# asbschmidt/CUDASW4

Measured on AMD Instinct MI355X. Metric: GCUPS, higher is better.
Workload: dtype f16x2; 1 GPU; peak: allqueries.fasta (20 queries, 41752 residues) vs pseudo DB 1000000 x 512, half2 kernel configuration, blosum62, gop -11 gex -1, top 10, C++ host driver; db_subjects=1000000, db_residues=512000000, queries=20, kernel=half2, queries_in_flight=1, tail_overlaps=10, numa_node_rank0=1, numa_bound=True, resident=True, residency=resident, cached_chars=512000000, parallelism=db-shard x1 (one DB sharded), one top-K gather per step + host merge

## Files before the change

cudasw4_amd/csrc/sw_api.hip:

```cpp
#include <hip/hip_runtime.h>
#include <hipcub/hipcub.hpp>

#include <algorithm>
#include <cstdio>
#include <cmath>
#include <cstdlib>
#include <cstring>
#include <ctime>
#include <string>
#include <vector>

#include "../../include/cudasw4_amd.h"
#include "../../include/cudasw4_amd_engine.h"
#include "../../include/cudasw4_amd_pssm.h"
#include "sw_internal.hpp"
#include "sw_launch.hpp"
#include "sw_pssm.hpp"
#include "sw_rows_pipeline.hpp"

namespace {

thread_local std::string g_last_error = "";

int fail(int code, const std::string& msg) {
// ... 122 lines not shown
    bool have_query = false;
    bool pssm_mode = false;
    int8_t* d_pssm = nullptr;
    size_t pssm_capacity = 0;
    int pssm_max = 1;
    Profile profiles[4][4][3];
    bool use_offs = true;
    int64_t long16_min = -1;
    int64_t long16_min_default = -1;
    int matrix_max = 1;
    bool i32_native = false;
    int32_t lanes4_max_subject = -1;
    int32_t lanes4_max_q = -1;
    int32_t lanes8_max_q = -1;
    bool check_bounds = false;
    uint32_t pipe_spin_limit = 1u << 20;
    int32_t pipe_drop_stage = -1;
    int32_t pipe_cpl = 0;
    int32_t stream_slots = 4;
    int32_t stream_jump = 0;
    int32_t stream_cols_max = 4096;
    int32_t stream_multi_cols_max = 1536;
    int32_t stream_multi_max_subject = -1;
    int32_t pipe_quorum = 0;
    int32_t pipe_slot = 0;
};

namespace {

int score_max(const sw_ctx* ctx) { return std::max(1, ctx->pssm_mode ? ctx->pssm_max : ctx->matrix_max); }
bool have_scores(const sw_ctx* ctx) { return ctx->have_matrix || ctx->pssm_mode; }

int max_grid(const sw_ctx* ctx) {
    const int g = std::max(1, ctx->num_cus) * ctx->grid_mult;
    return ctx->grid_cap > 0 ? std::min(g, ctx->grid_cap) : g;
}

int rescore_lanes(int32_t max_subject_len) { return max_subject_len > 1280 ? 64 : 16; }

int shape_index(int lanes) { return lanes == 64 ? 1 : lanes == 8 ? 2 : lanes == 4 ? 3 : 0; }

int effective_kind_of(const sw_ctx* ctx, int kind, int32_t max_subject_len) {
    if (kind != SW_KIND_I32 || ctx->i32_native || !ctx->have_query) return kind;
    const int64_t bound = (int64_t)std::min(ctx->qlen, max_subject_len) * score_max(ctx) + ((int64_t)1 << 22) + 4096;
    return bound < ((int64_t)1 << 24) ? SW_KIND_F32 : SW_KIND_I32;
}
// ... 39 lines not shown
        pr.dev = nullptr;
        pr.capacity = 0;
        SW_HIP(hipMalloc(&pr.dev, cap));
        pr.capacity = cap;
    }
    if (ctx->pssm_mode) SW_HIP(kl->profile(pl.rows, lanes, nullptr, ctx->qlen, ctx->d_pssm, ctx->qlen, pl.nstripes, pr.dev, shift, frame == 2 ? 1 : 0, stream));
    else SW_HIP(kl->profile(pl.rows, lanes, ctx->d_query, ctx->qlen, ctx->d_matrix, ctx->dim, pl.nstripes, pr.dev, shift, frame == 2 ? 1 : 0, stream));
    pr.shift = shift;
    if (!pr.ready) SW_HIP(hipEventCreateWithFlags(&pr.ready, hipEventDisableTiming));
    SW_HIP(hipEventRecord(pr.ready, stream));
    pr.plan = pl;
    pr.valid = true;
    return SW_OK;
}

int32_t border_capacity(int32_t max_len, int lanes) {
    const int64_t steps = ((int64_t)max_len + lanes - 1 + 3) / 4 * 4;
    return (int32_t)((steps + 15) / 16 * 16 + 16);
}
size_t border_bytes_per_wg(int32_t lcap, int lanes) {
    if (lanes == 4) return 0;
    const size_t region = lanes == 16 ? swk::group_region_words<16>(lcap) : lanes == 8 ? swk::group_region_words<8>(lcap) : swk::group_region_words<64>(lcap);
    return (size_t)(swk::kThreads / lanes) * region * sizeof(uint32_t);
}

__global__ void max_length_kernel(const int32_t* lengths, const int32_t* positions, const int32_t* count_ptr, int32_t first_pos,
                                  int32_t n, int32_t* out) {
    const int32_t cnt = count_ptr ? min(*count_ptr, n) : n;
    int32_t m = 0;
    for (int32_t i = blockIdx.x * blockDim.x + threadIdx.x; i < cnt; i += gridDim.x * blockDim.x)
        m = max(m, lengths[positions ? positions[i] : first_pos + i]);
    if (m > 0) atomicMax(out, m);
}

struct StreamPlan { int slots = 0, cols = 0, room = 0, base = 0, jump = 0; };
StreamPlan stream_plan(const sw_ctx* ctx, int kind, int lanes, int a, const QueryPlan& pl, int32_t max_subject_len) {
    StreamPlan sp;
    if (!kind_packed(kind) || lanes != 16 || a < 0) return sp;
    const bool multi = pl.nstripes > 1;
    const int P = swk::frame_classes(true, pl.rows, lanes, multi);
    sp.base = kind == SW_KIND_F16X2 ? -2016 : 0;
    const int top = kind == SW_KIND_F16X2 ? 1024 : 12400;
    sp.jump = ctx->stream_jump > 0 ? ctx->stream_jump : (kind == SW_KIND_F16X2 ? 512 : 2048);
    sp.room = top - sp.base - a * (2 * lanes + 4 + P);
    sp.cols = a > 0 ? std::min(sp.room / a, ctx->stream_cols_max) : ctx->stream_cols_max;
    sp.slots = std::max(1, std::min(ctx->stream_slots, swk::kStreamMaxSlots));
// ... 135 lines not shown
            p.uniform_frame = 1;
            for (int u = 0; u < swk::kLevelWords; u++)
                p.levels[u] = kind == SW_KIND_F16X2 ? swk::Arith<swk::F16X2>::zero_at(a, std::min<int>(u, (int)K + 16))
                                                    : swk::Arith<swk::I16X2>::zero_at(a, std::min<int>(u, (int)K + 16));
        }
    }
    if (sp.slots >= 1) {
        p.stream_slots = sp.slots; p.stream_cols = sp.cols; p.stream_room = sp.room; p.level_base = sp.base;
        p.jump = sp.jump; p.jump_limit = sp.jump - 4;
        p.jump_word = kind == SW_KIND_F16X2 ? swk::Arith<swk::F16X2>::pos_word(sp.jump) : swk::Arith<swk::I16X2>::pos_word(sp.jump);
    }
    p.scores = scores; p.ids = ids; p.id_offset = id_offset;
    p.ovf_pos = ovf_pos; p.ovf_count = ovf_count; p.ovf_check = (ovf_check && kind_packed(kind)) ? 1 : 0;
    p.scratch = nullptr; p.lcap = 0; p.zeros = ctx->d_zeros + kind * 16;
    p.stat_count = stat_count; p.stat_limit = stat_limit;
    if (multi) {
        p.lcap = border_capacity(max_subject_len, lanes);
        if (p.stream_slots > 1) {
            int cols = p.stream_cols;
            while (cols > max_subject_len && (size_t)grid * border_bytes_per_wg(border_capacity(cols, lanes), lanes) > temp_bytes) cols = cols * 3 / 4;
            p.stream_cols = cols;
            p.lcap = border_capacity(std::max(max_subject_len, cols), lanes);
        }
        const size_t per_wg = border_bytes_per_wg(p.lcap, lanes);
        if (!temp || temp_bytes < per_wg) return fail(SW_ERR_TEMP, "temp buffer too small for a multi-stripe query");
        grid = (int)std::min<size_t>((size_t)grid, temp_bytes / per_wg);
        p.scratch = static_cast<uint32_t*>(temp);
    }
    SW_HIP(take_work_slot(ctx, stream, &p.work_counter));
    p.start_signal = start_signal;
    p.start_quorum = (uint32_t)std::min(grid, 64);
    p.dry_signal = dry_signal;
    if (!stat_count && !positions && p.stream_slots > 1 && lanes == 16 && kind_packed(kind)) { p.stat_count = ctx->dirty_counter; p.stat_limit = INT32_MAX; }
    p.dry_value = ctx->dry_value;
    const int reserve = (list.service_workgroups > 0 || list.claim) ? 0 : ctx->grid_reserve;
    SW_HIP(kl->scan(pl.rows, lanes, multi, offs, grid, reserve, stream, p));
    return SW_OK;
}

}

namespace {
#define SW_REP8(OP) OP(0) OP(1) OP(2) OP(3) OP(4) OP(5) OP(6) OP(7)
#define SW_OP_PK_MAX3(i) asm volatile("v_pk_maximum3_f16 %0, %0, %1, %2" : "+v"(a[i]) : "v"(b), "v"(c));
#define SW_OP_ADD_F32(i) asm volatile("v_add_f32 %0, %0, %1" : "+v"(a[i]) : "v"(b));
#define SW_OP_MAX3_F32(i) asm volatile("v_max3_f32 %0, %0, %1, %2" : "+v"(a[i]) : "v"(b), "v"(c));
#define SW_OP_ADD_U32(i) asm volatile("v_add_u32 %0, %0, %1" : "+v"(a[i]) : "v"(b));
// ... 116 lines not shown
int sw_ctx_create(int device, sw_ctx** out) {
    if (!out) return fail(SW_ERR_INVALID, "null out pointer");
    *out = nullptr;
    int n = 0;
    if (hipGetDeviceCount(&n) != hipSuccess || n <= 0) return fail(SW_ERR_NO_DEVICE, "no HIP device available (this library has no CPU path)");
    if (device < 0 || device >= n) return fail(SW_ERR_INVALID, "device index out of range");
    SW_HIP(hipSetDevice(device));
    hipDeviceProp_t prop;
    SW_HIP(hipGetDeviceProperties(&prop, device));
    sw_ctx* ctx = new sw_ctx;
    ctx->device = device;
    ctx->num_cus = prop.multiProcessorCount;
    if (const char* e = getenv("CUDASW4_AMD_GRID_CAP")) ctx->grid_cap = std::max(0, atoi(e));
    if (const char* e = getenv("CUDASW4_AMD_NO_OFFS")) ctx->use_offs = !(e[0] == '1');
    if (const char* e = getenv("CUDASW4_AMD_I32_NATIVE")) ctx->i32_native = e[0] == '1';
    if (const char* e = getenv("CUDASW4_AMD_LANES8_MAX_Q")) ctx->lanes8_max_q = atoi(e);
    if (const char* e = getenv("CUDASW4_AMD_LANES4_MAX_Q")) ctx->lanes4_max_q = atoi(e);
    if (const char* e = getenv("CUDASW4_AMD_LANES4_MAX_SUBJECT")) ctx->lanes4_max_subject = atoi(e);
    if (const char* e = getenv("CUDASW4_AMD_CHECK_BOUNDS")) ctx->check_bounds = e[0] == '1';
    if (const char* e = getenv("CUDASW4_AMD_PIPE_SPIN_LIMIT")) ctx->pipe_spin_limit = (uint32_t)std::max(1ll, atoll(e));
    if (const char* e = getenv("CUDASW4_AMD_PIPE_TEST_DROP_STAGE")) ctx->pipe_drop_stage = atoi(e);
    if (const char* e = getenv("CUDASW4_AMD_PIPE_CPL")) ctx->pipe_cpl = atoi(e);
    if (const char* e = getenv("CUDASW4_AMD_STREAM")) ctx->stream_slots = std::max(0, std::min(swk::kStreamMaxSlots, atoi(e)));
    hipError_t e = hipMalloc(&ctx->d_matrix, 26 * swk::kLetters);
    if (e == hipSuccess) e = hipMalloc(&ctx->d_zeros, 256 + 64);
    if (e == hipSuccess) e = hipMalloc(&ctx->d_work, 2 * kWorkSlots * sizeof(uint32_t));
    if (e == hipSuccess) {
        uint32_t z[64] = {};
        for (int i = 0; i < 16; i++) z[SW_KIND_I16X2 * 16 + i] = swk::Arith<swk::I16X2>::kZero;
        e = hipMemcpy(ctx->d_zeros, z, sizeof(z), hipMemcpyHostToDevice);
    }
    for (int kind = 0; kind < 4 && e == hipSuccess; kind++) e = kind_launch(kind)->warm(nullptr);
    if (e == hipSuccess) e = hipStreamSynchronize(nullptr);
    if (e != hipSuccess) { delete ctx; return fail(SW_ERR_HIP, std::string("context set-up: ") + hipGetErrorString(e)); }
    *out = ctx;
    return SW_OK;
}

int sw_ctx_destroy(sw_ctx* ctx) {
    if (!ctx) return SW_OK;
    (void)hipSetDevice(ctx->device);
    if (ctx->d_matrix) (void)hipFree(ctx->d_matrix);
    if (ctx->d_zeros) (void)hipFree(ctx->d_zeros);
    if (ctx->d_work) (void)hipFree(ctx->d_work);
    if (ctx->d_query) (void)hipFree(ctx->d_query);
    if (ctx->d_pssm) (void)hipFree(ctx->d_pssm);
// ... 515 lines not shown
    return SW_OK;
}

static size_t scan_temp_bytes_of(sw_ctx* ctx, int kind, int part_id, int32_t n, int32_t max_subject_len);
size_t sw_scan_temp_bytes(sw_ctx* ctx, int kind, int part_id, int32_t n, int32_t max_subject_len) {
    if (!ctx || !ctx->have_query || !kind_launch(kind) || max_subject_len < 0 || n <= 0) return 0;
    if (kind_packed(kind) && part_id >= 0) {
        const int fb = packed_fallback_kind(kind);
        const size_t own = scan_temp_bytes_of(ctx, kind, part_id, n, max_subject_len);
        return std::max(own, scan_temp_bytes_of(ctx, effective_kind_of(ctx, fb, max_subject_len), part_id, n, max_subject_len));
    }
    return scan_temp_bytes_of(ctx, effective_kind_of(ctx, kind, max_subject_len), part_id, n, max_subject_len);
}

static size_t scan_temp_bytes_of(sw_ctx* ctx, int kind, int part_id, int32_t n, int32_t max_subject_len) {
    const int lanes = part_id < 0 ? rescore_lanes(max_subject_len) : lanes_for_partition(ctx, kind, part_id, n, max_subject_len);
    const QueryPlan pl = plan_query(kind, ctx->qlen, lanes);
    if (pl.nstripes <= 1) return 0;
    const int subj_per_batch = (swk::kThreads / lanes) * (kind_packed(kind) ? 2 : 1);
    const int64_t nbatches = ((int64_t)n + subj_per_batch - 1) / subj_per_batch;
    const int64_t grid = std::min<int64_t>(nbatches, max_grid(ctx));
    const StreamPlan sp = stream_plan(ctx, kind, lanes, 1, pl, max_subject_len);
    const int32_t cols = sp.slots > 1 ? std::max(max_subject_len, sp.cols) : max_subject_len;
    return (size_t)grid * border_bytes_per_wg(border_capacity(cols, lanes), lanes);
}

int sw_scan_partition(sw_ctx* ctx, int kind, int part_id, const int8_t* chars, const uint64_t* offsets,
                      const int32_t* lengths, int32_t first_pos, int32_t n, int32_t max_subject_len, int gop, int gex,
                      float* scores, int32_t* ids, int64_t id_offset, int32_t* ovf_pos, int32_t* ovf_count,
                      int ovf_check, void* temp, size_t temp_bytes, void* stream) {
    if (!ctx) return fail(SW_ERR_INVALID, "null context");
    if (part_id < 0 || part_id >= SW_NUM_LENGTH_PARTITIONS || !kind_launch(kind)) {
        ctx->start_signal = nullptr;
        ctx->dry_signal = nullptr;
        return fail(SW_ERR_INVALID, part_id < 0 || part_id >= SW_NUM_LENGTH_PARTITIONS ? "partition id out of range" : "unknown kind");
    }
    kind = effective_kind_of(ctx, kind, max_subject_len);
    int lanes = lanes_for_partition(ctx, kind, part_id, n, max_subject_len);
    if (kind_packed(kind) && !offs_possible(ctx, kind, lanes, max_subject_len, gop, gex, ovf_check, nullptr)) {
        kind = effective_kind_of(ctx, packed_fallback_kind(kind), max_subject_len);
        lanes = lanes_for_partition(ctx, kind, part_id, n, max_subject_len);
        ovf_pos = nullptr; ovf_count = nullptr; ovf_check = 0;
    }
    return scan_common(ctx, kind, lanes, chars, offsets, lengths, nullptr, nullptr, first_pos, n, max_subject_len, gop, gex,
                       scores, ids, id_offset, ovf_pos, ovf_count, ovf_check, temp, temp_bytes,
                       static_cast<hipStream_t>(stream));
// ... 471 lines not shown
```

cudasw4_amd/csrc/sw_dp_kernel.hpp:

```cpp
#pragma once

#include <hip/hip_runtime.h>
#include <stdint.h>

#include <type_traits>

#include "sw_pssm.hpp"

namespace swk {

typedef uint32_t u32;
typedef short s16x2 __attribute__((ext_vector_type(2)));
typedef unsigned short u16x2 __attribute__((ext_vector_type(2)));
typedef _Float16 f16x2 __attribute__((ext_vector_type(2)));

constexpr int kGroup = 16;
constexpr int kThreads = 256;
constexpr int kPadLetter = 20;
constexpr int kLetters = 21;

enum { F16X2 = 0, I16X2 = 1, I32 = 2, F32 = 3 };

constexpr int DPP_ROW_SHL1 = 0x101;
constexpr int DPP_ROW_SHR1 = 0x111;
// ... 261 lines not shown
    int32_t renorm_quads;
    u32 renorm_word;
    u32 wrap_class;
    u32 wrap_last;
    int32_t* stat_count;
    int32_t stat_limit;
    u32* start_signal;
    u32 start_quorum;
    int32_t* claim;
    int32_t service;
    const u32* done_flag;
    u32 done_value;
    u32* dry_signal;
    u32 dry_value;
    int32_t stream_slots;
    int32_t stream_cols;
    int32_t stream_room;
    int32_t level_base;
    int32_t jump;
    u32 jump_word;
    int32_t jump_limit;
    int32_t uniform_frame;
    int32_t flag_period;
    u32 levels[kLevelWords];
};

constexpr int32_t kListEmpty = -1, kListTaken = -2;

typedef u32 u32x3 __attribute__((ext_vector_type(3)));

template <int NW, int CHUNK_ROW_BYTES>
__device__ __forceinline__ void lds_read_chunk(u32 (&dst)[NW], const unsigned char* p, int c) {
    using C = Chunks<NW>;
    const int w = C::first(c);
    if (c < C::kN4) {
        const uint4 v = *reinterpret_cast<const uint4*>(p + c * CHUNK_ROW_BYTES);
        dst[w + 0] = v.x; dst[w + 1] = v.y; dst[w + 2] = v.z; dst[w + 3] = v.w;
    } else if (c < C::kCount) {
        const u32x3 v = *reinterpret_cast<const u32x3*>(p + c * CHUNK_ROW_BYTES);
        if constexpr (C::kSplit) {
            dst[w + 0] = v.x; dst[w + 1] = v.y; dst[w + 2] = v.z;
        } else {
            u32 x = v.x;
            if constexpr (C::kRem == 1) asm("" : "+v"(x) : "v"(v.y), "v"(v.z));
            if constexpr (C::kRem == 2) asm("" : "+v"(x) : "v"(v.z));
            dst[w] = x;
// ... 267 lines not shown
    return v;
}

template <int LANES>
struct Border {
    static constexpr int kBlockCols = 2 * LANES;
    static constexpr int kQuadsPerBlock = LANES / 2;
    static constexpr int kBlockBytes = 8 * kBlockCols;
    static constexpr int kBlockWords = 2 * kBlockCols;
    static constexpr int kInBytes = kBlockBytes, kOutBytes = kBlockBytes, kDummyBytes = 8 * (kThreads / LANES) + 32;
    static constexpr int kGroupBytes = kInBytes + kOutBytes + 16;
    static constexpr int ring_bytes(int groups) { return groups * kGroupBytes + kDummyBytes; }
    static_assert(kGroupBytes % 16 == 0, "rings are read and written 16 bytes at a time");
    static constexpr int blocks(int steps) { return (steps + kBlockCols - 1) / kBlockCols + 3; }
};
template <int LANES>
constexpr int border_region_words(int lcap) { return Border<LANES>::blocks(lcap) * Border<LANES>::kBlockWords; }

template <int LANES>
constexpr int stream_region_words(int lcap) { return LANES == 16 ? Border<LANES>::blocks(lcap) * Border<LANES>::kBlockCols : 0; }
template <int LANES>
constexpr int group_region_words(int lcap) { return border_region_words<LANES>(lcap) + stream_region_words<LANES>(lcap); }

__device__ __forceinline__ void announce_start(const ScanParams& p) {
    if (p.start_signal && threadIdx.x == 0) {
        if (atomicAdd(p.work_counter + 1, 1u) + 1u == p.start_quorum)
            __hip_atomic_fetch_add(p.start_signal, 1u, __ATOMIC_RELEASE, __HIP_MEMORY_SCOPE_SYSTEM);
    }
}

#ifndef SWK_I32_WAVES3_MAX_R
#define SWK_I32_WAVES3_MAX_R 32
#endif
#ifndef SWK_I32_WAVES3_MAX_R_MULTI
#define SWK_I32_WAVES3_MAX_R_MULTI 32
#endif
#ifndef SWK_F32_WAVES3_MAX_R
#define SWK_F32_WAVES3_MAX_R 48
#endif
#ifndef SWK_F32_WAVES3_MAX_R_MULTI
#define SWK_F32_WAVES3_MAX_R_MULTI 48
#endif
constexpr int min_waves_of(int KIND, int R, int LANES, bool MULTI) {
    const bool packed = KIND == F16X2 || KIND == I16X2;
    if (packed && LANES <= 16 && MULTI && R <= SWK_WAVES3_MAX_R_MULTI) return 3;
    if (packed) return (LANES <= 16 && !MULTI && R <= SWK_WAVES4_MAX_R) ? 4 : (LANES <= 16 && !MULTI && R <= SWK_WAVES3_MAX_R) ? 3 : 2;
    if (KIND == I32 && LANES <= 16 && R > (MULTI ? SWK_I32_WAVES3_MAX_R_MULTI : SWK_I32_WAVES3_MAX_R)) return 2;
    if (KIND == F32 && LANES <= 16 && R > (MULTI ? SWK_F32_WAVES3_MAX_R_MULTI : SWK_F32_WAVES3_MAX_R)) return 2;
    return (R <= 16 && !MULTI && LANES <= 16) ? 4 : 3;
}
template <int KIND, int R, int LANES, bool MULTI>
constexpr int min_waves() { return min_waves_of(KIND, R, LANES, MULTI); }
constexpr int vgpr_slot_of(int KIND, int R, int LANES, bool MULTI) { return (512 / min_waves_of(KIND, R, LANES, MULTI)) & ~7; }

template <int KIND, int R, int LANES, bool MULTI, bool OFFS = false>
__global__ void __launch_bounds__(kThreads, (min_waves<KIND, R, LANES, MULTI>())) sw_scan_kernel(const ScanParams p) {
    using A = Arith<KIND>;
    using G = Geometry<KIND, R, LANES>;
    constexpr int kGroups = kThreads / LANES;
    using BD = Border<LANES>;
    constexpr int SHL1 = Shift<LANES>::kShl1;
    constexpr int kQuadsPerLetterBlock = LANES;
    static_assert(!A::kPacked || OFFS, "packed kinds run the column-offset recurrence only (sw_launch.hpp: launch_scan_ro)");
    constexpr bool kUni = A::kPacked;
    constexpr bool kAddr = A::kPacked && MULTI && LANES == 16;
    constexpr int P = OFFS ? frame_classes(A::kPacked, R, LANES, MULTI, kUni) : 1;
    __shared__ __attribute__((aligned(16))) unsigned char lds[16 + G::kTileBytes];
    __shared__ __attribute__((aligned(16))) unsigned char rings[MULTI ? BD::ring_bytes(kGroups) : 16];

    const int tid = threadIdx.x;
    const int lane = tid & (LANES - 1);
    const int group = tid / LANES;
    const bool head = lane == 0;
    const int slot = LANES < 16 ? (tid & 15) : lane;
    const u32 laneStep = kAddr ? 16u * (u32)slot : (A::kPacked ? 0x00100010u : 16u) * ((LANES < 16 && head) ? u32(slot + 1) : 1u);
    announce_start(p);
    if (p.positions) __builtin_amdgcn_s_setprio(2);
    const bool service = p.service != 0;
    const int n = (p.count_ptr && !service) ? *p.count_ptr : p.n;
    constexpr int kSubjPerBatch = kGroups * A::kSubjects;
    const int nbatches = (n + kSubjPerBatch - 1) / kSubjPerBatch;
    if (!service && (int)blockIdx.x >= nbatches) return;

    if constexpr (!MULTI) {
        load_tile<G::kTileBytes>(lds, p.profile);
        __syncthreads();
    }

    unsigned char* const ringIn = rings + (MULTI ? group * BD::kGroupBytes : 0);
    unsigned char* const ringOut = ringIn + BD::kInBytes;
    u32* const gBorder = MULTI ? p.scratch + ((size_t)blockIdx.x * kGroups + group) * (size_t)group_region_words<LANES>(p.lcap) : nullptr;
    typedef const __attribute__((address_space(1))) unsigned char* StreamPtr;
    StreamPtr streamBase = nullptr;
    u32 streamOff = 0;
    if constexpr (kAddr) {
        constexpr int kGroupsPerWave = 64 / LANES;
        const int g0 = group & ~(kGroupsPerWave - 1);
        const uintptr_t b = reinterpret_cast<uintptr_t>(p.scratch + ((size_t)blockIdx.x * kGroups + g0) * (size_t)group_region_words<LANES>(p.lcap) +
                                                        border_region_words<LANES>(p.lcap));
        streamBase = (StreamPtr)(((uintptr_t)(u32)__builtin_amdgcn_readfirstlane((int)(b >> 32)) << 32) |
                                 (uintptr_t)(u32)__builtin_amdgcn_readfirstlane((int)(u32)b));
        streamOff = 4u * (u32)((group - g0) * group_region_words<LANES>(p.lcap) + LANES - lane);
    }

    const u32 apos = OFFS ? A::pos_word(p.gex_mag) : 0u;
// ... 8 lines not shown
        for (int spin = 0; spin < (1 << 20); spin++) {
            const int v = __hip_atomic_load(p.claim + i, __ATOMIC_RELAXED, __HIP_MEMORY_SCOPE_AGENT);
            if (v == kListTaken) return -1;
            if (v >= 0) return atomicCAS(p.claim + i, v, kListTaken) == v ? v : -1;
            __builtin_amdgcn_s_sleep(2);
        }
        return -1;
    };
    for (;;) {
        __syncthreads();
        if (tid == 0) {
            int b = (int)atomicAdd(p.work_counter, 1u), avail = n;
            if (service) {
                avail = 0;
                for (u32 spin = 0; b < nbatches; spin++) {
                    avail = __hip_atomic_load(p.count_ptr, __ATOMIC_RELAXED, __HIP_MEMORY_SCOPE_AGENT);
                    if (avail > b * kSubjPerBatch) break;
                    const u32 done = __hip_atomic_load(p.done_flag, __ATOMIC_RELAXED, __HIP_MEMORY_SCOPE_SYSTEM);
                    if ((int32_t)(done - p.done_value) >= 0 || spin > 600000u) { b = nbatches; break; }
                    __builtin_amdgcn_s_sleep(127);
                }
                avail = min(avail, n);
            }
            if (b == nbatches && p.dry_signal) __hip_atomic_store(p.dry_signal, p.dry_value, __ATOMIC_RELAXED, __HIP_MEMORY_SCOPE_SYSTEM);
            next_batch = b;
            batch_avail = avail;
        }
        __syncthreads();
        const int b = next_batch;
        if (b >= nbatches) break;
        const int navail = batch_avail;
        const int batch = service ? b : nbatches - 1 - b;
        const int i0 = batch * kSubjPerBatch + group * A::kSubjects;
        const int i1 = i0 + 1;
        bool valid0 = i0 < navail;
        bool valid1 = A::kPacked && (i1 < navail);
        int pos0 = 0, pos1 = 0, len0 = 0, len1 = 0;
        const int8_t* s0 = p.chars;
        const int8_t* s1 = p.chars;
        if (p.claim) {
            int v = -1;
            if (valid0 && lane == 0) v = claim_entry(i0);
            if constexpr (LANES == 64) v = __builtin_amdgcn_readfirstlane(v);
            else v = __shfl(v, (tid & 63) & ~(LANES - 1));
            valid0 = v >= 0;
            pos0 = valid0 ? v : 0;
            if (valid0) {
                len0 = p.lengths[pos0];
                s0 = p.chars + (p.offsets[pos0] - p.offsets[0]);
            }
            valid1 = false;
        } else {
            if (valid0) {
                pos0 = p.positions ? p.positions[i0] : p.first_pos + i0;
                len0 = p.lengths[pos0];
                s0 = p.chars + (p.offsets[pos0] - p.offsets[0]);
            }
            if (valid1) {
                pos1 = p.positions ? p.positions[i1] : p.first_pos + i1;
                len1 = p.lengths[pos1];
                s1 = p.chars + (p.offsets[pos1] - p.offsets[0]);
            }
        }
        int lmax = len0 > len1 ? len0 : len1;
        if constexpr (LANES <= 16) {
            if constexpr (LANES <= 4) lmax = max(lmax, __shfl_xor(lmax, 4));
            if constexpr (LANES <= 8) lmax = max(lmax, __shfl_xor(lmax, 8));
            lmax = max(lmax, __shfl_xor(lmax, 16));
            lmax = max(lmax, __shfl_xor(lmax, 32));
        }
        int nquads = (lmax + LANES - 1 + 3) >> 2;
        if constexpr (MULTI) nquads = min(nquads, (p.lcap - 4) >> 2);
        nquads = __builtin_amdgcn_readfirstlane(nquads);
        const int len0pad = (len0 + 3) & ~3, len1pad = (len1 + 3) & ~3;
        auto letters4 = [&](const int8_t* s, int lenpad, int j) -> u32 {
            u32 w = 0x14141414u;
            if (j < lenpad) w = *reinterpret_cast<const u32*>(s + j);
            return w * (u32)G::kLetterUnits;
        };
        if constexpr (kAddr) {
            u32* const sw = gBorder + border_region_words<LANES>(p.lcap) + LANES;
            sw[lane - LANES] = (u32)(kPadLetter * G::kLetterUnits) * 0x01000100u;
            for (int c = lane; c < nquads + LANES / 4; c += LANES) {
                const u32 a = letters4(s0, len0pad, 4 * c), b = letters4(s1, len1pad, 4 * c);
                *reinterpret_cast<uint4*>(sw + 4 * c) = make_uint4(__builtin_amdgcn_perm(b, a, 0x040c000cu), __builtin_amdgcn_perm(b, a, 0x050c010cu),
                                                                   __builtin_amdgcn_perm(b, a, 0x060c020cu), __builtin_amdgcn_perm(b, a, 0x070c030cu));
            }
            __builtin_amdgcn_fence(__ATOMIC_RELEASE, "workgroup");
        }

        u32 maxv = 0u;
        for (int stripe = 0; stripe < p.nstripes; stripe++) {
            const bool first = stripe == 0;
            if constexpr (MULTI) {
                __syncthreads();
                load_tile<G::kTileBytes>(lds, p.profile + (size_t)stripe * G::kTileBytes);
                __syncthreads();
            }
            StripeState<KIND, R, P> st;
            u32 zw[P + 5];
            const int tg0 = kUni ? __builtin_amdgcn_readfirstlane(LANES * stripe) : 0;
            auto load_levels = [&](int q) {
                const int u0 = __builtin_amdgcn_readfirstlane((tg0 + 4 * q) & kmask);
#pragma unroll
                for (int k = 0; k < P + 5; k++) zw[k] = p.levels[u0 + k];
#pragma unroll
                for (int k = 0; k < P + 5; k++) asm volatile("" : "+s"(zw[k]));
            };
            if constexpr (kUni) {
                load_levels(0);
#pragma unroll
                for (int r = 0; r < R; r++) { st.H[r] = zw[r % P]; st.E[r] = zw[r % P + 1]; }
                st.upH_prev = A::gap(zw[(R - 1) % P], p.gex); st.Hlast = zw[(R - 1) % P]; st.Fout = zw[0];
#pragma unroll
                for (int d = 0; d < P + 3; d++) st.maxv[d] = A::add(maxv, zw[d + 1]);
            } else {
                u32 zc[P + 5];
                zc[0] = zbefore; zc[1] = zstart;
#pragma unroll
                for (int k = 2; k < P + 5; k++) zc[k] = A::add(zc[k - 1], apos);
#pragma unroll
                for (int r = 0; r < R; r++) { st.H[r] = zc[r % P]; st.E[r] = zc[r % P + 1]; }
                st.upH_prev = zc[(R - 1) % P]; st.Hlast = zc[(R - 1) % P]; st.Fout = zbefore;
#pragma unroll
                for (int k = 0; k < P + 4; k++) st.Zc[k] = zc[k + 1];
#pragma unroll
                for (int d = 0; d < P + 3; d++) st.maxv[d] = OFFS ? A::add(maxv, zc[A::kWindow ? d + 1 : d]) : maxv;
            }
            st.yA = ((u32)(kPadLetter * G::kLetterUnits) << G::kLetterShift) + 16u * (u32)(slot + 1);
            st.yB = st.yA;
            if constexpr (A::kPacked && LANES <= 16) st.yA |= st.yA << 16;

            auto fetch = [&](const int8_t* s, int lenpad, int blk) -> u32 {
                if constexpr (kAddr) return 0u;
                else return letters4(s, lenpad, blk * (4 * LANES) + lane * 4);
            };
            u32 nextA = fetch(s0, len0pad, 0);
            u32 nextB = A::kPacked ? fetch(s1, len1pad, 0) : 0u;
// ... 105 lines not shown
                        if (lower) lower_frame();
                    }
                    if constexpr (MULTI) *reinterpret_cast<uint2*>(outPtr + 8 * BYTE) = make_uint2(st.Hlast, st.Fout);
                };
                border_step(std::integral_constant<int, 0>{});
                border_step(std::integral_constant<int, 1>{});
                border_step(std::integral_constant<int, 2>{});
                border_step(std::integral_constant<int, 3>{});
                if constexpr (MULTI) outPtr += walkOut;
                if constexpr (!kAddr) {
                    lettersA = dpp<SHL1, true>(0u, lettersA);
                    if constexpr (A::kPacked) lettersB = dpp<SHL1, true>(0u, lettersB);
                }
                if constexpr (OFFS && A::kWindow) {
                    if constexpr (!kUni) {
#pragma unroll
                        for (int k = 0; k < P + 4; k++) st.Zc[k] = A::add(st.Zc[k], apos4);
                    }
#pragma unroll
                    for (int d = 0; d < P + 3; d++) st.maxv[d] = A::add(st.maxv[d], apos4);
                }
                if constexpr (kUni) load_levels(q + 1);
            };
            if constexpr (!MULTI) {
                for (int q = 0; q < nquads; q++) quad(q);
            } else {
                for (int q0 = 0; q0 < nquads; q0 += BD::kQuadsPerBlock) {
                    const int qend = min(nquads, q0 + BD::kQuadsPerBlock);
                    for (int q = q0; q < qend; q++) quad(q);
                    if (qend == q0 + BD::kQuadsPerBlock) block_end(q0 / BD::kQuadsPerBlock);
                }
            }
            if constexpr (MULTI) {
                if (!last) {
                    const int done = nquads & ~(BD::kQuadsPerBlock - 1);
                    const int slot = 4 * (nquads - done) + lane;
                    u32* const g = gBorder + (size_t)(done / BD::kQuadsPerBlock) * BD::kBlockWords;
                    __builtin_amdgcn_fence(__ATOMIC_ACQ_REL, "wavefront");
                    if (slot < BD::kBlockCols) *reinterpret_cast<uint2*>(ringOut + 8 * slot) = make_uint2(A::kZero, A::kZero);
                    else *reinterpret_cast<uint2*>(g + 2 * slot) = make_uint2(A::kZero, A::kZero);
                    __builtin_amdgcn_fence(__ATOMIC_ACQ_REL, "wavefront");
                    *reinterpret_cast<uint4*>(g + 4 * lane) = *reinterpret_cast<const uint4*>(ringOut + 16 * lane);
                }
            }
            if constexpr (kUni) {
                maxv = A::true_of(st.maxv[0], zw[1]);
#pragma unroll
                for (int d = 1; d < P + 3; d++) maxv = A::true_max(maxv, A::true_of(st.maxv[d], zw[d + 1]));
            } else if constexpr (OFFS) {
                if constexpr (A::kWindow) {
                    maxv = A::true_of(st.maxv[0], st.Zc[0]);
#pragma unroll
                    for (int d = 1; d < P + 3; d++) maxv = A::true_max(maxv, A::true_of(st.maxv[d], st.Zc[d]));
                } else {
                    maxv = A::true_of(st.maxv[0], A::gap(A::gap(st.Zc[1], p.gex), p.gex));
#pragma unroll
                    for (int c = 1; c < P; c++)
                        maxv = A::true_max(maxv, A::true_of(st.maxv[c], A::gap(A::gap(st.Zc[c + 1], p.gex), p.gex)));
                }
            } else {
                maxv = st.maxv[0];
            }
            if constexpr (MULTI) __builtin_amdgcn_fence(__ATOMIC_RELEASE, "workgroup");
        }

        int sc0, sc1, guard = 0;
        if constexpr (OFFS) {
            if constexpr (LANES == 8) {
                maxv = half_row_max(maxv, [](u32 a, u32 b) { return A::true_max(a, b); });
            } else if constexpr (LANES == 4) {
                maxv = quad_max(maxv, [](u32 a, u32 b) { return A::true_max(a, b); });
            } else {
                maxv = row_max_true<KIND>(maxv);
            }
            if constexpr (LANES == 64) {
                maxv = A::true_max(maxv, (u32)__shfl_xor((int)maxv, 16));
                maxv = A::true_max(maxv, (u32)__shfl_xor((int)maxv, 32));
            }
            sc0 = A::true_lo(maxv);
            sc1 = A::true_hi(maxv);
            if constexpr (kUni) {
                const int tgmax = 4 * nquads + LANES * (p.nstripes - 1);
                constexpr int kColP = frame_classes(true, R, LANES, MULTI);
                guard = max(p.gex_mag * ((tgmax > 4 * rq ? 4 * rq : tgmax) + P + 8),
                            p.gex_mag * (min(4 * nquads, p.flag_period) + 2 * LANES + 4 + kColP));
            } else {
                guard = p.gex_mag * (4 * nquads + 2 * LANES + 4 + P);
            }
        } else {
            maxv = group_max<KIND, LANES>(maxv);
            sc0 = A::score_lo(maxv);
            sc1 = 0;
        }
        if (lane == 0) {
            if (valid0) {
                if (A::kPacked && p.ovf_check && sc0 >= A::kLimit - guard) {
                    __hip_atomic_store(p.ovf_pos + atomicAdd(p.ovf_count, 1), pos0, __ATOMIC_RELAXED, __HIP_MEMORY_SCOPE_AGENT);
                } else {
                    p.scores[pos0] = (float)sc0;
                    if (p.stat_count && sc0 >= p.stat_limit) atomicAdd(p.stat_count, 1);
                }
                p.ids[pos0] = (int32_t)(p.id_offset + pos0);
            }
            if (valid1) {
                if (p.ovf_check && sc1 >= A::kLimit - guard) {
                    __hip_atomic_store(p.ovf_pos + atomicAdd(p.ovf_count, 1), pos1, __ATOMIC_RELAXED, __HIP_MEMORY_SCOPE_AGENT);
                } else {
                    p.scores[pos1] = (float)sc1;
                }
                p.ids[pos1] = (int32_t)(p.id_offset + pos1);
            }
        }
    }
}

template <int KIND, int R, int LANES>
__global__ void sw_build_profile_kernel(const int8_t* __restrict__ query, int32_t qlen,
                                        const int8_t* __restrict__ matrix21, int32_t pad_row, int32_t nstripes,
                                        unsigned char* __restrict__ profile, int32_t shift, int32_t head_extra) {
    using A = Arith<KIND>;
    using G = Geometry<KIND, R, LANES>;
    constexpr int kWordsPerRow = G::kRowBytes / 4;
    constexpr int kWordsPerChunkRow = G::kChunkRowBytes / 4;
    const size_t total = (size_t)nstripes * kLetters * kWordsPerRow;
    u32* out = reinterpret_cast<u32*>(profile);
    for (size_t i = (size_t)blockIdx.x * blockDim.x + threadIdx.x; i < total; i += (size_t)gridDim.x * blockDim.x) {
        const int word = (int)(i % kWordsPerRow);
        const int letter = (int)((i / kWordsPerRow) % kLetters);
        const int stripe = (int)(i / ((size_t)kWordsPerRow * kLetters));
        const int chunk = word / kWordsPerChunkRow, lane = ((word % kWordsPerChunkRow) / 4) % LANES, sub = word % 4;
        const int w = G::C::first(chunk) + sub;
        u32 v = 0;
        if (sub < G::C::words(chunk) && w < G::NW) {
            auto entry = [&](int row_in_lane) -> u32 {
// ... 20 lines not shown
```

Measured before the change: 12070 GCUPS.

## Chain multiple subject batches into one multi-stripe DP pass per workgroup

For packed 16-lane multi-stripe queries with short subjects, each workgroup concatenates up to three subject pairs along the column axis and runs them as one long DP sweep. Lanes reset their state at chain boundaries, and per-segment maxima are kept in scratch. This amortises the per-batch stripe-pass overhead, including the border/ring handoff, pipeline fill and drain, and profile reload, across several short subjects. The cost is extra scratch memory, padding columns between subjects, reset logic inside the quad loop, and more complex overflow-guard bookkeeping.

```diff
diff --git a/cudasw4_amd/csrc/sw_api.hip b/cudasw4_amd/csrc/sw_api.hip
--- a/cudasw4_amd/csrc/sw_api.hip
+++ b/cudasw4_amd/csrc/sw_api.hip
@@ -168,6 +168,8 @@
     int32_t stream_cols_max = 4096;
     int32_t stream_multi_cols_max = 1536;
     int32_t stream_multi_max_subject = -1;
+    int32_t chain = 3;
+    bool chain_all = false;
     int32_t pipe_quorum = 0;
     int32_t pipe_slot = 0;
 };
@@ -253,6 +255,22 @@
     if (lanes == 4) return 0;
     const size_t region = lanes == 16 ? swk::group_region_words<16>(lcap) : lanes == 8 ? swk::group_region_words<8>(lcap) : swk::group_region_words<64>(lcap);
     return (size_t)(swk::kThreads / lanes) * region * sizeof(uint32_t);
+}
+
+constexpr int kChainMinRounds = 16;
+constexpr int32_t kChainMaxSubject = 1024;
+int chain_wanted(const sw_ctx* ctx, int kind, int lanes, bool multi, int stream_slots, int64_t nbatches, int32_t max_subject_len) {
+    if (!kind_packed(kind) || lanes != 16 || !multi || stream_slots != 1) return 1;
+    if (ctx->chain <= 1 || max_subject_len > kChainMaxSubject) return 1;
+    if (!ctx->chain_all && nbatches <= (int64_t)std::max(ctx->chain, kChainMinRounds) * max_grid(ctx)) return 1;
+    return std::min<int>(ctx->chain, swk::kChainMax);
+}
+int32_t chain_capacity(int32_t max_len, int chain, int lanes) {
+    return border_capacity((int32_t)std::min<int64_t>(swk::chain_columns(max_len, chain), SW_MAX_SUBJECT_LEN), lanes);
+}
+size_t chain_bytes_per_wg(int32_t max_len, int chain, int lanes) {
+    if (chain <= 1) return border_bytes_per_wg(border_capacity(max_len, lanes), lanes);
+    return border_bytes_per_wg(chain_capacity(max_len, chain, lanes), lanes) + (size_t)(swk::kThreads / lanes) * swk::kChainMaxWords * sizeof(uint32_t);
 }
 
 __global__ void max_length_kernel(const int32_t* lengths, const int32_t* positions, const int32_t* count_ptr, int32_t first_pos,
@@ -434,7 +452,15 @@
             p.stream_cols = cols;
             p.lcap = border_capacity(std::max(max_subject_len, cols), lanes);
         }
-        const size_t per_wg = border_bytes_per_wg(p.lcap, lanes);
+        int chain = (positions || count_ptr || list.claim || list.service_workgroups > 0) ? 1
+                        : chain_wanted(ctx, kind, lanes, multi, p.stream_slots, nbatches, max_subject_len);
+        while (chain > 1 && (size_t)grid * chain_bytes_per_wg(max_subject_len, chain, lanes) > temp_bytes) chain--;
+        if (chain > 1) {
+            p.chain = chain;
+            p.chain_all = ctx->chain_all ? 1 : 0;
+            p.lcap = chain_capacity(max_subject_len, chain, lanes);
+        }
+        const size_t per_wg = chain > 1 ? chain_bytes_per_wg(max_subject_len, chain, lanes) : border_bytes_per_wg(p.lcap, lanes);
         if (!temp || temp_bytes < per_wg) return fail(SW_ERR_TEMP, "temp buffer too small for a multi-stripe query");
         grid = (int)std::min<size_t>((size_t)grid, temp_bytes / per_wg);
         p.scratch = static_cast<uint32_t*>(temp);
@@ -597,6 +623,8 @@
     if (const char* e = getenv("CUDASW4_AMD_PIPE_TEST_DROP_STAGE")) ctx->pipe_drop_stage = atoi(e);
     if (const char* e = getenv("CUDASW4_AMD_PIPE_CPL")) ctx->pipe_cpl = atoi(e);
     if (const char* e = getenv("CUDASW4_AMD_STREAM")) ctx->stream_slots = std::max(0, std::min(swk::kStreamMaxSlots, atoi(e)));
+    if (const char* e = getenv("CUDASW4_AMD_CHAIN")) ctx->chain = std::max(1, std::min(swk::kChainMax, atoi(e)));
+    if (const char* e = getenv("CUDASW4_AMD_CHAIN_ALL")) ctx->chain_all = e[0] == '1';
     hipError_t e = hipMalloc(&ctx->d_matrix, 26 * swk::kLetters);
     if (e == hipSuccess) e = hipMalloc(&ctx->d_zeros, 256 + 64);
     if (e == hipSuccess) e = hipMalloc(&ctx->d_work, 2 * kWorkSlots * sizeof(uint32_t));
@@ -1158,6 +1186,8 @@
     const int64_t grid = std::min<int64_t>(nbatches, max_grid(ctx));
     const StreamPlan sp = stream_plan(ctx, kind, lanes, 1, pl, max_subject_len);
     const int32_t cols = sp.slots > 1 ? std::max(max_subject_len, sp.cols) : max_subject_len;
+    const int chain = part_id < 0 ? 1 : chain_wanted(ctx, kind, lanes, true, sp.slots, nbatches, max_subject_len);
+    if (chain > 1) return (size_t)grid * chain_bytes_per_wg(max_subject_len, chain, lanes);
     return (size_t)grid * border_bytes_per_wg(border_capacity(cols, lanes), lanes);
 }
 
diff --git a/cudasw4_amd/csrc/sw_dp_kernel.hpp b/cudasw4_amd/csrc/sw_dp_kernel.hpp
--- a/cudasw4_amd/csrc/sw_dp_kernel.hpp
+++ b/cudasw4_amd/csrc/sw_dp_kernel.hpp
@@ -307,6 +307,8 @@
     int32_t jump_limit;
     int32_t uniform_frame;
     int32_t flag_period;
+    int32_t chain;
+    int32_t chain_all;
     u32 levels[kLevelWords];
 };
 
@@ -620,6 +622,12 @@
 template <int LANES>
 constexpr int group_region_words(int lcap) { return border_region_words<LANES>(lcap) + stream_region_words<LANES>(lcap); }
 
+constexpr int kChainMax = 8;
+constexpr int kChainMinCols = 12;
+constexpr int kChainMaxWords = (kChainMax - 1) * kGroup;
+constexpr int chain_pair_columns(int lmax) { return ((lmax + 3) & ~3) < kChainMinCols ? kChainMinCols : ((lmax + 3) & ~3); }
+constexpr int64_t chain_columns(int max_len, int c) { return (int64_t)(c - 1) * (chain_pair_columns(max_len) + 4) + max_len; }
+
 __device__ __forceinline__ void announce_start(const ScanParams& p) {
     if (p.start_signal && threadIdx.x == 0) {
         if (atomicAdd(p.work_counter + 1, 1u) + 1u == p.start_quorum)
@@ -662,8 +670,10 @@
     static_assert(!A::kPacked || OFFS, "packed kinds run the column-offset recurrence only (sw_launch.hpp: launch_scan_ro)");
     constexpr bool kUni = A::kPacked;
     constexpr bool kAddr = A::kPacked && MULTI && LANES == 16;
+    constexpr bool kChain = kAddr;
     constexpr int P = OFFS ? frame_classes(A::kPacked, R, LANES, MULTI, kUni) : 1;
     __shared__ __attribute__((aligned(16))) unsigned char lds[16 + G::kTileBytes];
+    __shared__ int chainEnd[kChain ? (kThreads / 64) * kChainMax : 1];
     __shared__ __attribute__((aligned(16))) unsigned char rings[MULTI ? BD::ring_bytes(kGroups) : 16];
 
     const int tid = threadIdx.x;
@@ -679,6 +689,9 @@
     constexpr int kSubjPerBatch = kGroups * A::kSubjects;
     const int nbatches = (n + kSubjPerBatch - 1) / kSubjPerBatch;
     if (!service && (int)blockIdx.x >= nbatches) return;
+    const int kC = kChain ? min(max(p.chain, 1), kChainMax) : 1;
+    const int nchain = (!kChain || kC == 1) ? 0 : p.chain_all ? (nbatches + kC - 1) / kC : max(0, (nbatches - kC * (int)gridDim.x + kC - 1) / kC);
+    const int nclaims = kChain ? nchain + max(0, nbatches - nchain * kC) : nbatches;
 
     if constexpr (!MULTI) {
         load_tile<G::kTileBytes>(lds, p.profile);
@@ -733,54 +746,77 @@
                 }
                 avail = min(avail, n);
             }
-            if (b == nbatches && p.dry_signal) __hip_atomic_store(p.dry_signal, p.dry_value, __ATOMIC_RELAXED, __HIP_MEMORY_SCOPE_SYSTEM);
+            if (b == nclaims && p.dry_signal) __hip_atomic_store(p.dry_signal, p.dry_value, __ATOMIC_RELAXED, __HIP_MEMORY_SCOPE_SYSTEM);
             next_batch = b;
             batch_avail = avail;
         }
         __syncthreads();
         const int b = next_batch;
-        if (b >= nbatches) break;
+        if (b >= nclaims) break;
         const int navail = batch_avail;
-        const int batch = service ? b : nbatches - 1 - b;
-        const int i0 = batch * kSubjPerBatch + group * A::kSubjects;
-        const int i1 = i0 + 1;
-        bool valid0 = i0 < navail;
-        bool valid1 = A::kPacked && (i1 < navail);
-        int pos0 = 0, pos1 = 0, len0 = 0, len1 = 0;
-        const int8_t* s0 = p.chars;
-        const int8_t* s1 = p.chars;
-        if (p.claim) {
-            int v = -1;
-            if (valid0 && lane == 0) v = claim_entry(i0);
-            if constexpr (LANES == 64) v = __builtin_amdgcn_readfirstlane(v);
-            else v = __shfl(v, (tid & 63) & ~(LANES - 1));
-            valid0 = v >= 0;
-            pos0 = valid0 ? v : 0;
-            if (valid0) {
-                len0 = p.lengths[pos0];
-                s0 = p.chars + (p.offsets[pos0] - p.offsets[0]);
-            }
-            valid1 = false;
-        } else {
-            if (valid0) {
-                pos0 = p.positions ? p.positions[i0] : p.first_pos + i0;
-                len0 = p.lengths[pos0];
-                s0 = p.chars + (p.offsets[pos0] - p.offsets[0]);
-            }
-            if (valid1) {
-                pos1 = p.positions ? p.positions[i1] : p.first_pos + i1;
-                len1 = p.lengths[pos1];
-                s1 = p.chars + (p.offsets[pos1] - p.offsets[0]);
-            }
-        }
-        int lmax = len0 > len1 ? len0 : len1;
-        if constexpr (LANES <= 16) {
-            if constexpr (LANES <= 4) lmax = max(lmax, __shfl_xor(lmax, 4));
-            if constexpr (LANES <= 8) lmax = max(lmax, __shfl_xor(lmax, 8));
-            lmax = max(lmax, __shfl_xor(lmax, 16));
-            lmax = max(lmax, __shfl_xor(lmax, 32));
-        }
-        int nquads = (lmax + LANES - 1 + 3) >> 2;
+        int hb = b, cnt = 1;
+        if constexpr (kChain) {
+            if (b < nchain) { hb = kC * b; cnt = min(kC, nbatches - hb); }
+            else hb = nchain * kC + (b - nchain);
+            hb = __builtin_amdgcn_readfirstlane(hb);
+            cnt = __builtin_amdgcn_readfirstlane(cnt);
+        }
+        struct Pair {
+            bool valid0 = false, valid1 = false;
+            int pos0 = 0, pos1 = 0, len0 = 0, len1 = 0, lmax = 0;
+            const int8_t* s0 = nullptr;
+            const int8_t* s1 = nullptr;
+        };
+        auto load_pair = [&](int hbk) -> Pair {
+            Pair r;
+            const int batch = service ? hbk : nbatches - 1 - hbk;
+            const int i0 = batch * kSubjPerBatch + group * A::kSubjects;
+            const int i1 = i0 + 1;
+            r.valid0 = i0 < navail;
+            r.valid1 = A::kPacked && (i1 < navail);
+            r.s0 = p.chars;
+            r.s1 = p.chars;
+            if (p.claim) {
+                int v = -1;
+                if (r.valid0 && lane == 0) v = claim_entry(i0);
+                if constexpr (LANES == 64) v = __builtin_amdgcn_readfirstlane(v);
+                else v = __shfl(v, (tid & 63) & ~(LANES - 1));
+                r.valid0 = v >= 0;
+                r.pos0 = r.valid0 ? v : 0;
+                if (r.valid0) {
+                    r.len0 = p.lengths[r.pos0];
+                    r.s0 = p.chars + (p.offsets[r.pos0] - p.offsets[0]);
+                }
+                r.valid1 = false;
+            } else {
+                if (r.valid0) {
+                    r.pos0 = p.positions ? p.positions[i0] : p.first_pos + i0;
+                    r.len0 = p.lengths[r.pos0];
+                    r.s0 = p.chars + (p.offsets[r.pos0] - p.offsets[0]);
+                }
+                if (r.valid1) {
+                    r.pos1 = p.positions ? p.positions[i1] : p.first_pos + i1;
+                    r.len1 = p.lengths[r.pos1];
+                    r.s1 = p.chars + (p.offsets[r.pos1] - p.offsets[0]);
+                }
+            }
+            int lmax = r.len0 > r.len1 ? r.len0 : r.len1;
+            if constexpr (LANES <= 16) {
+                if constexpr (LANES <= 4) lmax = max(lmax, __shfl_xor(lmax, 4));
+                if constexpr (LANES <= 8) lmax = max(lmax, __shfl_xor(lmax, 8));
+                lmax = max(lmax, __shfl_xor(lmax, 16));
+                lmax = max(lmax, __shfl_xor(lmax, 32));
+            }
+            r.lmax = lmax;
+            return r;
+        };
+        Pair pr;
+        if constexpr (!kChain) pr = load_pair(hb);
+        const bool valid0 = pr.valid0, valid1 = pr.valid1;
+        const int pos0 = pr.pos0, pos1 = pr.pos1, len0 = pr.len0, len1 = pr.len1;
+        const int8_t* const s0 = pr.s0;
+        const int8_t* const s1 = pr.s1;
+        int nquads = (pr.lmax + LANES - 1 + 3) >> 2;
         if constexpr (MULTI) nquads = min(nquads, (p.lcap - 4) >> 2);
         nquads = __builtin_amdgcn_readfirstlane(nquads);
         const int len0pad = (len0 + 3) & ~3, len1pad = (len1 + 3) & ~3;
@@ -791,12 +827,26 @@
         };
         if constexpr (kAddr) {
             u32* const sw = gBorder + border_region_words<LANES>(p.lcap) + LANES;
+            const int wcap = 4 * ((p.lcap - 4) >> 2) + LANES;
             sw[lane - LANES] = (u32)(kPadLetter * G::kLetterUnits) * 0x01000100u;
-            for (int c = lane; c < nquads + LANES / 4; c += LANES) {
-                const u32 a = letters4(s0, len0pad, 4 * c), b = letters4(s1, len1pad, 4 * c);
-                *reinterpret_cast<uint4*>(sw + 4 * c) = make_uint4(__builtin_amdgcn_perm(b, a, 0x040c000cu), __builtin_amdgcn_perm(b, a, 0x050c010cu),
-                                                                   __builtin_amdgcn_perm(b, a, 0x060c020cu), __builtin_amdgcn_perm(b, a, 0x070c030cu));
-            }
+            auto put4 = [&](const Pair& q, int col0, int c) {
+                if (col0 + 4 * c + 4 > wcap) return;
+                const u32 a = letters4(q.s0, (q.len0 + 3) & ~3, 4 * c), b = letters4(q.s1, (q.len1 + 3) & ~3, 4 * c);
+                *reinterpret_cast<uint4*>(sw + col0 + 4 * c) = make_uint4(__builtin_amdgcn_perm(b, a, 0x040c000cu), __builtin_amdgcn_perm(b, a, 0x050c010cu),
+                                                                          __builtin_amdgcn_perm(b, a, 0x060c020cu), __builtin_amdgcn_perm(b, a, 0x070c030cu));
+            };
+            int col0 = 0;
+            for (int k = 0; k + 1 < cnt; k++) {
+                const Pair q = load_pair(hb + k);
+                const int T = chain_pair_columns(__builtin_amdgcn_readfirstlane(q.lmax));
+                for (int c = lane; c < T / 4 + 1; c += LANES) put4(q, col0, c);
+                if ((tid & 63) == 0) chainEnd[(tid >> 6) * kChainMax + k] = col0 + T;
+                col0 += T + 4;
+            }
+            const Pair q = load_pair(hb + cnt - 1);
+            nquads = (col0 + __builtin_amdgcn_readfirstlane(q.lmax) + LANES - 1 + 3) >> 2;
+            nquads = __builtin_amdgcn_readfirstlane(min(nquads, (p.lcap - 4) >> 2));
+            for (int c = lane; c < nquads - col0 / 4 + LANES / 4; c += LANES) put4(q, col0, c);
             __builtin_amdgcn_fence(__ATOMIC_RELEASE, "workgroup");
         }
 
@@ -823,8 +873,9 @@
 #pragma unroll
                 for (int r = 0; r < R; r++) { st.H[r] = zw[r % P]; st.E[r] = zw[r % P + 1]; }
                 st.upH_prev = A::gap(zw[(R - 1) % P], p.gex); st.Hlast = zw[(R - 1) % P]; st.Fout = zw[0];
-#pragma unroll
-                for (int d = 0; d < P + 3; d++) st.maxv[d] = A::add(maxv, zw[d + 1]);
+                const u32 seed = (kChain && cnt > 1) ? 0u : maxv;
+#pragma unroll
+                for (int d = 0; d < P + 3; d++) st.maxv[d] = A::add(seed, zw[d + 1]);
             } else {
                 u32 zc[P + 5];
                 zc[0] = zbefore; zc[1] = zstart;
@@ -976,8 +1027,51 @@
                 }
                 if constexpr (kUni) load_levels(q + 1);
             };
+            auto reset_lanes = [&](int k, int j) {
+                if constexpr (kChain) {
+                    int t = tid;
+                    asm volatile("" : "+v"(t));
+                    const int ln = t & (LANES - 1), grp = t / LANES;
+                    if ((ln >> 2) == j) {
+                        u32 m = A::true_of(st.maxv[0], zw[1]);
+#pragma unroll
+                        for (int d = 1; d < P + 3; d++) m = A::true_max(m, A::true_of(st.maxv[d], zw[d + 1]));
+                        u32* const pm = p.scratch + (size_t)gridDim.x * kGroups * (size_t)group_region_words<LANES>(p.lcap) +
+                                        ((size_t)blockIdx.x * kGroups + grp) * kChainMaxWords + kGroup * k + ln;
+                        if (!first) m = A::true_max(m, *pm);
+                        *pm = m;
+#pragma unroll
+                        for (int d = 0; d < P + 3; d++) st.maxv[d] = zw[d + 1];
+#pragma unroll
+                        for (int r = 0; r < R; r++) { st.H[r] = zw[r % P]; st.E[r] = zw[r % P + 1]; }
+                        st.upH_prev = A::gap(zw[(R - 1) % P], p.gex); st.Hlast = zw[(R - 1) % P]; st.Fout = zw[0];
+                    }
+                }
+            };
             if constexpr (!MULTI) {
                 for (int q = 0; q < nquads; q++) quad(q);
+            } else if constexpr (kChain) {
+                constexpr int kNever = 0x7fffffff;
+                const int* const ends = chainEnd + (tid >> 6) * kChainMax;
+                int rk = 0, rj = 0;
+                int nextReset = cnt > 1 ? __builtin_amdgcn_readfirstlane((ends[0] >> 2) + 1) : kNever;
+                for (int q0 = 0; q0 < nquads; q0 += BD::kQuadsPerBlock) {
+                    const int qend = min(nquads, q0 + BD::kQuadsPerBlock);
+                    int q = q0;
+                    for (;;) {
+                        const int seg = min(qend, nextReset);
+                        for (; q < seg; q++) quad(q);
+                        if (q >= qend) break;
+                        reset_lanes(rk, rj);
+                        nextReset++;
+                        if (++rj == 4) {
+                            rj = 0;
+                            rk++;
+                            nextReset = rk + 1 < cnt ? __builtin_amdgcn_readfirstlane((ends[rk] >> 2) + 1) : kNever;
+                        }
+                    }
+                    if (qend == q0 + BD::kQuadsPerBlock) block_end(q0 / BD::kQuadsPerBlock);
+                }
             } else {
                 for (int q0 = 0; q0 < nquads; q0 += BD::kQuadsPerBlock) {
                     const int qend = min(nquads, q0 + BD::kQuadsPerBlock);
@@ -998,9 +1092,13 @@
                 }
             }
             if constexpr (kUni) {
+                const u32 above = maxv;
                 maxv = A::true_of(st.maxv[0], zw[1]);
 #pragma unroll
                 for (int d = 1; d < P + 3; d++) maxv = A::true_max(maxv, A::true_of(st.maxv[d], zw[d + 1]));
+                if constexpr (kChain) {
+                    if (cnt > 1) maxv = A::true_max(maxv, above);
+                }
             } else if constexpr (OFFS) {
                 if constexpr (A::kWindow) {
                     maxv = A::true_of(st.maxv[0], st.Zc[0]);
@@ -1018,52 +1116,72 @@
             if constexpr (MULTI) __builtin_amdgcn_fence(__ATOMIC_RELEASE, "workgroup");
         }
 
-        int sc0, sc1, guard = 0;
-        if constexpr (OFFS) {
-            if constexpr (LANES == 8) {
-                maxv = half_row_max(maxv, [](u32 a, u32 b) { return A::true_max(a, b); });
-            } else if constexpr (LANES == 4) {
-                maxv = quad_max(maxv, [](u32 a, u32 b) { return A::true_max(a, b); });
+        auto finish = [&](bool valid0, bool valid1, int pos0, int pos1, u32 maxv, int nq, int col0) {
+            int sc0, sc1, guard = 0;
+            if constexpr (OFFS) {
+                if constexpr (LANES == 8) {
+                    maxv = half_row_max(maxv, [](u32 a, u32 b) { return A::true_max(a, b); });
+                } else if constexpr (LANES == 4) {
+                    maxv = quad_max(maxv, [](u32 a, u32 b) { return A::true_max(a, b); });
+                } else {
+                    maxv = row_max_true<KIND>(maxv);
+                }
+                if constexpr (LANES == 64) {
+                    maxv = A::true_max(maxv, (u32)__shfl_xor((int)maxv, 16));
+                    maxv = A::true_max(maxv, (u32)__shfl_xor((int)maxv, 32));
+                }
+                sc0 = A::true_lo(maxv);
+                sc1 = A::true_hi(maxv);
+                if constexpr (kUni) {
+                    const int tgmax = 4 * nq + col0 + LANES * (p.nstripes - 1);
+                    constexpr int kColP = frame_classes(true, R, LANES, MULTI);
+                    guard = max(p.gex_mag * ((tgmax > 4 * rq ? 4 * rq : tgmax) + P + 8),
+                                p.gex_mag * (min(4 * nq, p.flag_period) + 2 * LANES + 4 + kColP));
+                } else {
+                    guard = p.gex_mag * (4 * nq + 2 * LANES + 4 + P);
+                }
             } else {
-                maxv = row_max_true<KIND>(maxv);
-            }
-            if constexpr (LANES == 64) {
-                maxv = A::true_max(maxv, (u32)__shfl_xor((int)maxv, 16));
-                maxv = A::true_max(maxv, (u32)__shfl_xor((int)maxv, 32));
-            }
-            sc0 = A::true_lo(maxv);
-            sc1 = A::true_hi(maxv);
-            if constexpr (kUni) {
-                const int tgmax = 4 * nquads + LANES * (p.nstripes - 1);
-                constexpr int kColP = frame_classes(true, R, LANES, MULTI);
-                guard = max(p.gex_mag * ((tgmax > 4 * rq ? 4 * rq : tgmax) + P + 8),
-                            p.gex_mag * (min(4 * nquads, p.flag_period) + 2 * LANES + 4 + kColP));
-            } else {
-                guard = p.gex_mag * (4 * nquads + 2 * LANES + 4 + P);
+                maxv = group_max<KIND, LANES>(maxv);
+                sc0 = A::score_lo(maxv);
+                sc1 = 0;
+            }
+            if (lane == 0) {
+                if (valid0) {
+                    if (A::kPacked && p.ovf_check && sc0 >= A::kLimit - guard) {
+                        __hip_atomic_store(p.ovf_pos + atomicAdd(p.ovf_count, 1), pos0, __ATOMIC_RELAXED, __HIP_MEMORY_SCOPE_AGENT);
+                    } else {
+                        p.scores[pos0] = (float)sc0;
+                        if (p.stat_count && sc0 >= p.stat_limit) atomicAdd(p.stat_count, 1);
+                    }
+                    p.ids[pos0] = (int32_t)(p.id_offset + pos0);
+                }
+                if (valid1) {
+                    if (p.ovf_check && sc1 >= A::kLimit - guard) {
+                        __hip_atomic_store(p.ovf_pos + atomicAdd(p.ovf_count, 1), pos1, __ATOMIC_RELAXED, __HIP_MEMORY_SCOPE_AGENT);
+                    } else {
+                        p.scores[pos1] = (float)sc1;
+                    }
+                    p.ids[pos1] = (int32_t)(p.id_offset + pos1);
+                }
+            }
+        };
+        if constexpr (kChain) {
+            int col0 = 0;
+            for (int k = 0; k < cnt; k++) {
+                const Pair q = load_pair(hb + k);
+                const int lm = __builtin_amdgcn_readfirstlane(q.lmax);
+                const bool lastPair = k + 1 == cnt;
+                int t = tid;
+                asm volatile("" : "+v"(t));
+                const u32* const pm = p.scratch + (size_t)gridDim.x * kGroups * (size_t)group_region_words<LANES>(p.lcap) +
+                                      ((size_t)blockIdx.x * kGroups + t / LANES) * kChainMaxWords + kGroup * k + (t & (LANES - 1));
+                u32 m = maxv;
+                if (!lastPair) m = *pm;
+                finish(q.valid0, q.valid1, q.pos0, q.pos1, m, lastPair ? nquads - col0 / 4 : (lm + LANES - 1 + 3) >> 2, col0);
+                col0 += chain_pair_columns(lm) + 4;
             }
         } else {
-            maxv = group_max<KIND, LANES>(maxv);
-            sc0 = A::score_lo(maxv);
-            sc1 = 0;
-        }
-        if (lane == 0) {
-            if (valid0) {
-                if (A::kPacked && p.ovf_check && sc0 >= A::kLimit - guard) {
-                    __hip_atomic_store(p.ovf_pos + atomicAdd(p.ovf_count, 1), pos0, __ATOMIC_RELAXED, __HIP_MEMORY_SCOPE_AGENT);
-                } else {
-                    p.scores[pos0] = (float)sc0;
-                    if (p.stat_count && sc0 >= p.stat_limit) atomicAdd(p.stat_count, 1);
-                }
-                p.ids[pos0] = (int32_t)(p.id_offset + pos0);
-            }
-            if (valid1) {
-                if (p.ovf_check && sc1 >= A::kLimit - guard) {
-                    __hip_atomic_store(p.ovf_pos + atomicAdd(p.ovf_count, 1), pos1, __ATOMIC_RELAXED, __HIP_MEMORY_SCOPE_AGENT);
-                } else {
-                    p.scores[pos1] = (float)sc1;
-                }
-                p.ids[pos1] = (int32_t)(p.id_offset + pos1);
-            }
+            finish(valid0, valid1, pos0, pos1, maxv, nquads, 0);
         }
     }
 }
```

Result: faster. 12220 GCUPS, median of 6 (+1.2%).
